# Leonhard111/M3L

Hardware: AMD Instinct MI355X
Metric: MAE fwd+bwd samples/sec (image+tactile) (higher is better)
Workload: dtype bf16; 1 GPU; BASELINE configs[1]: VTT vision+tactile MAE, 64x64 RGB + 2x32x32 tactile, ViT-Tiny 192/12/3/768 + decoder 192/4/3/768, mask 0.75; batch_per_gpu=256, global_batch=256, parallelism=dp1, grad_allreduce=none (one rank), rccl_ranks=0, step=zero_grad + mask + fwd + bwd + grad all-reduce + Adam

## Files before the change

include/m3l_amd.h:

```cpp
#ifndef M3L_AMD_H
#define M3L_AMD_H
#include <stddef.h>
#include <stdint.h>

#ifdef __cplusplus
extern "C" {
#endif

#define M3L_MAX_TACTILES 8

typedef struct m3l_geom {
    int image_h, image_w, image_patch, image_channels;
    int tactile_h, tactile_w, tactile_patch, tactile_channels;
    int num_tactiles;
    int use_vision;
    int use_tactile;
} m3l_geom;

typedef struct m3l_tf_cfg {
    int dim, depth, heads, mlp_dim;
    int project_out;
    int dtype;
    int dim_head;
} m3l_tf_cfg;
// ... 174 lines not shown
int m3l_prof_count(void);
int m3l_prof_get(int i, char* name, size_t n, double* ms_total, long* launches, double* flops_total, double* bytes_total);

int m3l_op_gemm_nt(int dtype, const void* A, int lda, const void* W, int ldw, int M, int N, int K, const float* bias,
                   const float* res, float* out_f32, void* out_t, void* out_pre, const void* gelu_u, int act, int ldc, void* stream);
size_t m3l_op_gemm_tn_ws_bytes(int M, int N, int K);
int m3l_op_gemm_tn(int dtype, const void* Y, int ldy, const void* X, int ldx, int M, int N, int K, void* ws, size_t ws_bytes,
                   float* out, int ldo, void* stream);
int m3l_op_gemm_tn_acc(int dtype, const void* Y, int ldy, const void* X, int ldx, int M, int N, int K, void* ws, size_t ws_bytes, float* out, int ldo,
                       int accumulate, void* stream);
size_t m3l_op_gemm_tn_grouped_ws_bytes(int dtype, int count, int M, const int* N, const int* K);
int m3l_op_gemm_tn_grouped(int dtype, int count, int M, const void* const* Y, const int* ldy, const void* const* X, const int* ldx, const int* N,
                           const int* K, float* const* out, void* ws, size_t ws_bytes, void* stream);
size_t m3l_op_colsum_ws_bytes(int N);
int m3l_op_colsum(int dtype, const void* Y, int M, int N, int ld, void* ws, float* out, void* stream);
int m3l_op_prep_weight(int dtype, const float* src, int rows, int cols, void* dst, void* dstT, void* stream);
int m3l_op_mask_scale(int mode, const float* src, const void* ref, float scale, long count, float* out, void* stream);
int m3l_op_concat2(float* a, int na, float* b, int nb, int rows, float* cat, int split, void* stream);
int m3l_op_patch_cols(int dtype, const float* x, int B, int C, int H, int W, int P, int Kpad, void* col, void* stream);
int m3l_op_vit_tokens(const float* emb, const float* cls, const float* regs, const float* pos, int B, int npatch, int R, int D, float* tok,
                      void* stream);
int m3l_op_attn_fwd(int dtype, const void* qkv, void* o, float* lse, int B, int n, int H, void* stream);
int m3l_op_attn_bwd(int dtype, const void* qkv, const void* o, const void* dO, const float* lse, float* dsum, void* dqkv, int B,
                    int n, int H, void* stream);
int m3l_op_attn_fwd_dh(int dtype, const void* qkv, void* o, float* lse, int B, int n, int H, void* stream, int dim_head);
int m3l_op_attn_bwd_dh(int dtype, const void* qkv, const void* o, const void* dO, const float* lse, float* dsum, void* dqkv, int B,
                       int n, int H, void* stream, int dim_head);
int m3l_op_dropout_mask(float p, uint64_t seed, int layer, int site, long rows, int N, uint8_t* out, void* stream);

int m3l_op_l2norm_fwd(int out_dtype, const float* x, int M, int D, float eps, void* y, float* y32, float* norm, void* stream);
// ... 34 lines not shown
```

m3l_amd/_lib.py:

```python
import ctypes as C
import os

_HERE = os.path.dirname(os.path.abspath(__file__))
LIB_PATH = os.environ.get("M3L_LIB_PATH") or os.path.join(_HERE, "lib", "libm3l_amd.so")

c_p = C.c_void_p
c_i = C.c_int
c_sz = C.c_size_t


class Geom(C.Structure):
    _fields_ = [(n, c_i) for n in ("image_h", "image_w", "image_patch", "image_channels", "tactile_h", "tactile_w",
                                   "tactile_patch", "tactile_channels", "num_tactiles", "use_vision", "use_tactile")]


class CnnCfg(C.Structure):
    _fields_ = [(n, c_i) for n in ("in_channels", "height", "width", "dim", "tactile", "dtype")]


class TfCfg(C.Structure):
    _fields_ = [(n, c_i) for n in ("dim", "depth", "heads", "mlp_dim", "project_out", "dtype", "dim_head")]


class MaeCfg(C.Structure):
# ... 92 lines not shown
    "m3l_adamw_step": (c_i, [c_p, c_p, c_p, c_p, C.c_long, C.c_float, C.c_float, C.c_float, C.c_float, C.c_float, c_i, C.c_float, C.c_float, c_p, c_i, c_p]),
    "m3l_adam_step": (c_i, [c_p, c_p, c_p, c_p, C.c_long, C.c_float, C.c_float, C.c_float, C.c_float, C.c_float, c_i, c_p]),
    "m3l_adam_step_scaled": (c_i, [c_p, c_p, c_p, c_p, C.c_long, C.c_float, C.c_float, C.c_float, C.c_float, C.c_float, c_i, C.c_float, c_p]),
    "m3l_dino_opt_step": (c_i, [c_p, c_p, c_p, c_p, c_p, C.c_long, c_p, c_p, c_i, C.POINTER(C.c_float), C.POINTER(C.c_float), c_i,
                                C.c_double, C.c_double, C.c_float, c_i, C.c_float, C.c_float, c_p, c_i, C.c_double, c_p]),
    "m3l_prof_begin": (None, [C.c_char_p, c_i]),
    "m3l_prof_end": (None, []),
    "m3l_prof_event_overhead_us": (C.c_double, [c_p, c_i]),
    "m3l_prof_count": (c_i, []),
    "m3l_prof_get": (c_i, [c_i, C.c_char_p, c_sz, C.POINTER(C.c_double), C.POINTER(C.c_long), C.POINTER(C.c_double),
                           C.POINTER(C.c_double)]),
    "m3l_op_gemm_nt": (c_i, [c_i, c_p, c_i, c_p, c_i, c_i, c_i, c_i, c_p, c_p, c_p, c_p, c_p, c_p, c_i, c_i, c_p]),
    "m3l_op_gemm_tn_ws_bytes": (c_sz, [c_i, c_i, c_i]),
    "m3l_op_gemm_tn": (c_i, [c_i, c_p, c_i, c_p, c_i, c_i, c_i, c_i, c_p, c_sz, c_p, c_i, c_p]),
    "m3l_op_gemm_tn_acc": (c_i, [c_i, c_p, c_i, c_p, c_i, c_i, c_i, c_i, c_p, c_sz, c_p, c_i, c_i, c_p]),
    "m3l_op_gemm_tn_grouped_ws_bytes": (c_sz, [c_i, c_i, c_i, c_p, c_p]),
    "m3l_op_gemm_tn_grouped": (c_i, [c_i, c_i, c_i, c_p, c_p, c_p, c_p, c_p, c_p, c_p, c_p, c_sz, c_p]),
    "m3l_op_colsum_ws_bytes": (c_sz, [c_i]),
    "m3l_op_colsum": (c_i, [c_i, c_p, c_i, c_i, c_i, c_p, c_p, c_p]),
    "m3l_op_prep_weight": (c_i, [c_i, c_p, c_i, c_i, c_p, c_p, c_p]),
    "m3l_op_mask_scale": (c_i, [c_i, c_p, c_p, C.c_float, C.c_long, c_p, c_p]),
    "m3l_op_concat2": (c_i, [c_p, c_i, c_p, c_i, c_i, c_p, c_i, c_p]),
    "m3l_op_patch_cols": (c_i, [c_i, c_p, c_i, c_i, c_i, c_i, c_i, c_i, c_p, c_p]),
    "m3l_op_vit_tokens": (c_i, [c_p, c_p, c_p, c_p, c_i, c_i, c_i, c_i, c_p, c_p]),
    "m3l_op_attn_fwd": (c_i, [c_i, c_p, c_p, c_p, c_i, c_i, c_i, c_p]),
    "m3l_op_attn_bwd": (c_i, [c_i, c_p, c_p, c_p, c_p, c_p, c_p, c_i, c_i, c_i, c_p]),
    "m3l_op_attn_fwd_dh": (c_i, [c_i, c_p, c_p, c_p, c_i, c_i, c_i, c_p, c_i]),
    "m3l_op_attn_bwd_dh": (c_i, [c_i, c_p, c_p, c_p, c_p, c_p, c_p, c_i, c_i, c_i, c_p, c_i]),
    "m3l_op_dropout_mask": (c_i, [C.c_float, C.c_uint64, c_i, c_i, C.c_long, c_i, c_p, c_p]),
    "m3l_op_l2norm_fwd": (c_i, [c_i, c_p, c_i, c_i, C.c_float, c_p, c_p, c_p, c_p]),
# ... 70 lines not shown
```

m3l_amd/csrc/elementwise.hip:

```cpp
#include "common.cuh"
#include "kernels.h"
#include <cstring>
#include <vector>

namespace {

constexpr int MAXV = 16;
constexpr int WPB = 4;

__device__ __forceinline__ void store_val(float* p, float v) { *p = v; }
__device__ __forceinline__ void store_val(bf16* p, float v) { *p = (bf16)v; }


template <typename TO> __device__ __forceinline__ void store4(TO* p, f32x4 v);
template <> __device__ __forceinline__ void store4<float>(float* p, f32x4 v) { *reinterpret_cast<f32x4*>(p) = v; }
template <> __device__ __forceinline__ void store4<bf16>(bf16* p, f32x4 v) {
    bf16x4 o;
    o[0] = (bf16)v[0]; o[1] = (bf16)v[1]; o[2] = (bf16)v[2]; o[3] = (bf16)v[3];
    *reinterpret_cast<bf16x4*>(p) = o;
}
__device__ __forceinline__ f32x4 load4(const float* p) { return *reinterpret_cast<const f32x4*>(p); }
__device__ __forceinline__ f32x4 load4(const bf16* p) {
    const bf16x4 v = *reinterpret_cast<const bf16x4*>(p);
    return f32x4{(float)v[0], (float)v[1], (float)v[2], (float)v[3]};
// ... 108 lines not shown
        if (256 * i >= D) break;
        *reinterpret_cast<f32x4*>(&red[wave][0][4 * lane]) = dg[i];
        *reinterpret_cast<f32x4*>(&red[wave][1][4 * lane]) = db[i];
        *reinterpret_cast<f32x4*>(&red[wave][2][4 * lane]) = dc[i];
        __syncthreads();
        const int e = 256 * i + threadIdx.x;
        if (e < D) {
#pragma unroll
            for (int k = 0; k < 3; ++k)
                out[k * D + e] = (red[0][k][threadIdx.x] + red[1][k][threadIdx.x]) + (red[2][k][threadIdx.x] + red[3][k][threadIdx.x]);
        }
        __syncthreads();
    }
}

__device__ __forceinline__ void reduce_cols_32x32(const float* __restrict__ p, int G, int stride, int j, bool valid,
                                                  float* __restrict__ out, int accumulate) {
    __shared__ float red[32][33];
    const int cl = threadIdx.x & 31, sl = threadIdx.x >> 5;
    float s = 0.f;
    if (valid) {
        float a[8] = {0.f, 0.f, 0.f, 0.f, 0.f, 0.f, 0.f, 0.f};
        int g = sl;
        for (; g + 224 < G; g += 256) {
#pragma unroll
            for (int u = 0; u < 8; ++u) a[u] += p[(long)(g + 32 * u) * stride + j];
        }
        for (; g < G; g += 32) a[0] += p[(long)g * stride + j];
        s = ((a[0] + a[1]) + (a[2] + a[3])) + ((a[4] + a[5]) + (a[6] + a[7]));
    }
    red[sl][cl] = s;
    __syncthreads();
    if (sl == 0 && valid) {
        float t = red[0][cl];
#pragma unroll
        for (int i = 1; i < 32; ++i) t += red[i][cl];
        out[j] = accumulate ? out[j] + t : t;
    }
}

__global__ __launch_bounds__(1024) void reduce_rows_kernel(const float* __restrict__ part, int G, int stride, int count,
                                                             float* __restrict__ out, int accumulate) {
    const int j = blockIdx.x * 32 + (threadIdx.x & 31);
    reduce_cols_32x32(part, G, stride, j, j < count, out, accumulate);
}

__global__ __launch_bounds__(1024) void reduce_vec_kernel(const float* __restrict__ v, int G, float* __restrict__ out, int accumulate) {
    __shared__ float red[16];
    float a0 = 0.f, a1 = 0.f, a2 = 0.f, a3 = 0.f;
    int i = threadIdx.x;
    for (; i + 3072 < G; i += 4096) { a0 += v[i]; a1 += v[i + 1024]; a2 += v[i + 2048]; a3 += v[i + 3072]; }
    for (; i < G; i += 1024) a0 += v[i];
    float s = wave_sum((a0 + a1) + (a2 + a3));
    if ((threadIdx.x & 63) == 0) red[threadIdx.x >> 6] = s;
    __syncthreads();
    if (threadIdx.x == 0) {
        float t = 0.f;
#pragma unroll
        for (int w = 0; w < 16; ++w) t += red[w];
        out[0] = accumulate ? out[0] + t : t;
    }
}

struct ReduceSegs { float* out[4]; };
__global__ __launch_bounds__(1024) void reduce_rows_seg_kernel(const float* __restrict__ part, int G, int stride, int width,
                                                                 ReduceSegs segs, int accumulate) {
    float* out = segs.out[blockIdx.y];
    if (!out) return;
    const int j = blockIdx.x * 32 + (threadIdx.x & 31);
    reduce_cols_32x32(part + (long)blockIdx.y * width, G, stride, j, j < width, out, accumulate);
}

__global__ __launch_bounds__(1024) void reduce_rows_batch_kernel(ReduceBatch b, int accumulate) {
    const ReduceBatchItem it = b.it[blockIdx.z];
    float* out = it.out[blockIdx.y];
    if (!out) return;
    const int j = blockIdx.x * 32 + (threadIdx.x & 31);
    reduce_cols_32x32(it.part + (long)blockIdx.y * b.D, it.G, 3 * b.D, j, j < b.D, out, accumulate);
}

template <typename T> struct Vec4;
template <> struct Vec4<bf16> { typedef bf16x4 type; };
template <> struct Vec4<float> { typedef f32x4 type; };
template <typename T>
__global__ __launch_bounds__(256) void colsum_kernel(const T* __restrict__ Y, int M, int N, int ld, int rows_per_block,
                                                       float* __restrict__ part, int vec_ok) {
    typedef typename Vec4<T>::type V4;
    const int r0 = blockIdx.x * rows_per_block, r1 = min(M, r0 + rows_per_block);
    for (int c = threadIdx.x * 4; c < N; c += 1024) {
        if (vec_ok && c + 4 <= N) {
            f32x4 s0 = f32x4{0.f, 0.f, 0.f, 0.f}, s1 = s0, s2 = s0, s3 = s0;
            auto ld4 = [&](int r) {
                const V4 v = *reinterpret_cast<const V4*>(Y + (long)r * ld + c);
// ... 1025 lines not shown
        else { if (D <= 256) LN_FWD(float, 1, bf16); else if (D <= 512) LN_FWD(float, 2, bf16); else LN_FWD(float, 4, bf16); }
    } else if (out_dtype == 1) {
        if (D <= 256) LN_FWD(bf16, 1, float); else if (D <= 512) LN_FWD(bf16, 2, float); else LN_FWD(bf16, 4, float);
    } else {
        if (D <= 256) LN_FWD(float, 1, float); else if (D <= 512) LN_FWD(float, 2, float); else LN_FWD(float, 4, float);
    }
#undef LN_FWD
    M3L_LAUNCH_CHECK();
    return 0;
}

int m3l_reduce_rows(const float* part, int G, int stride, int count, float* out, int accumulate, hipStream_t st) {
    if (count == 1 && stride == 1)
        reduce_vec_kernel<<<1, 1024, 0, st>>>(part, G, out, accumulate);
    else
        reduce_rows_kernel<<<cdiv(count, 32), 1024, 0, st>>>(part, G, stride, count, out, accumulate);
    M3L_LAUNCH_CHECK();
    return 0;
}

int m3l_ln_bwd_blocks(int M) {
    static const int forced = getenv("M3L_LN_ROWS_PER_WAVE") ? atoi(getenv("M3L_LN_ROWS_PER_WAVE")) : 0;
    const int rpw = forced > 0 ? forced : (M >= 12288 ? 4 : std::max(1, M / 4096));
    int G = cdiv(M, rpw * WPB);
    if (G > 2048) G = 2048;
    return G < 1 ? 1 : G;
}

int m3l_ln_bwd(int dy_dtype, const void* dy, const float* x, int M, int D, const float* gamma, float eps, const float* dres,
               float* dx_out, void* dx_t_out, int ct_dtype, float* part_ws, float* dgamma, float* dbeta, float* dbias,
               int accumulate, hipStream_t st) {
// ... 5 lines not shown
#define LN_BWD(TD, TC, C, TX) ln_bwd_kernel<TD, TC, C, TX><<<G, 256, 0, st>>>((const TD*)dy, (const TX*)x, M, D, gamma, eps, dres, dx_out, (TC*)dx_t_out, part_ws)
#define LN_BWD_C(TD, TC, TX) { if (D <= 256) LN_BWD(TD, TC, 1, TX); else if (D <= 512) LN_BWD(TD, TC, 2, TX); else LN_BWD(TD, TC, 4, TX); }
        if (m3l_call_rb()) {
            M3L_CHECK(!dx_out && dx_t_out && ct_dtype == 1, "ln_bwd: bf16 residual mode writes the compute-type gradient only");
            if (dy_dtype == 1) LN_BWD_C(bf16, bf16, bf16) else LN_BWD_C(float, bf16, bf16)
        }
        else if (dy_dtype == 1) LN_BWD_C(bf16, bf16, float)
        else if (ct_dtype == 1) LN_BWD_C(float, bf16, float)
        else LN_BWD_C(float, float, float)
#undef LN_BWD_C
#undef LN_BWD
    }
    M3L_LAUNCH_CHECK();
    if (!dgamma && !dbeta && !dbias) return 0;
    ReduceSegs segs = {{dgamma, dbeta, dbias, nullptr}};
    reduce_rows_seg_kernel<<<dim3(cdiv(D, 32), 3), 1024, 0, st>>>(part_ws, G, 3 * D, D, segs, accumulate);
    M3L_LAUNCH_CHECK();
    return 0;
}

int m3l_reduce_rows_batch(const ReduceBatch* b, int accumulate, hipStream_t st) {
    if (b->count <= 0) return 0;
    M3L_CHECK(b->count <= M3L_REDUCE_BATCH_MAX && b->D > 0, "reduce_rows_batch: count=%d D=%d", b->count, b->D);
    ProfScope prof("reduce_batch", b->count, b->D, 0, 0.0, st);
    reduce_rows_batch_kernel<<<dim3(cdiv(b->D, 32), 3, b->count), 1024, 0, st>>>(*b, accumulate);
    M3L_LAUNCH_CHECK();
    return 0;
}

int m3l_reduce_rows_seg3(const float* part, int G, int D, float* out0, float* out1, float* out2, int accumulate, hipStream_t st) {
    ReduceSegs segs = {{out0, out1, out2, nullptr}};
    reduce_rows_seg_kernel<<<dim3(cdiv(D, 32), 3), 1024, 0, st>>>(part, G, 3 * D, D, segs, accumulate);
    M3L_LAUNCH_CHECK();
    return 0;
}

int m3l_colsum(int dtype, const void* Y, int M, int N, int ld, float* part_ws, float* out, int accumulate, hipStream_t st) {
    M3L_CHECK(M > 0 && N > 0, "colsum: bad shape");
    int G = cdiv(M, N > 512 ? 16 : 64);
    if (G > m3l_part_blocks()) G = m3l_part_blocks();
    const int rpb = cdiv(M, G);
    G = cdiv(M, rpb);
    ProfScope prof("colsum", M, N, dtype, (double)M * N * (dtype ? 2 : 4), st);
    const int vec_ok = (ld % 4 == 0) && (N % 4 == 0) && (((unsigned long)Y) % 16 == 0) && (((unsigned long)part_ws) % 16 == 0);
    if (dtype == 1)
        colsum_kernel<bf16><<<G, 256, 0, st>>>((const bf16*)Y, M, N, ld, rpb, part_ws, vec_ok);
    else
// ... 137 lines not shown
int k_tokens_assemble(const float* img_tok, const float* tac_tok, int B, int D, int n_img, int n_tac, int k, const float* mod,
                        const float* pos_img, const float* pos_tac, float* tokens, hipStream_t st) {
    const long rows = (long)B * (n_img + k * n_tac);
    tokens_assemble_kernel<<<cdiv(rows, WPB), 256, 0, st>>>(img_tok, tac_tok, B, D, n_img, n_tac > 0 ? n_tac : 1, k, mod, pos_img, pos_tac, tokens);
    M3L_LAUNCH_CHECK();
    return 0;
}

int k_tokens_assemble_bwd(const float* dtok, int B, int D, int n_img, int n_tac, int k, float* d_img, float* d_tac, float* part_ws,
                            float* dmod, int accumulate, hipStream_t st) {
    const long rows = (long)B * (n_img + k * n_tac);
    const int PL = (1 + k) * D;
    const int G = part_grid(rows);
    tokens_assemble_bwd_kernel<<<G, 256, WPB * PL * sizeof(float), st>>>(dtok, B, D, n_img, n_tac > 0 ? n_tac : 1, k, d_img, d_tac, part_ws);
    M3L_LAUNCH_CHECK();
    reduce_rows_kernel<<<cdiv(PL, 32), 1024, 0, st>>>(part_ws, G, PL, PL, dmod, accumulate);
    M3L_LAUNCH_CHECK();
    return 0;
}

int m3l_adam_flat(float* p, const float* g, float* m, float* v, long n, float lr, float b1, float b2, float eps, float wd, int step,
                  float gscale, hipStream_t st) {
    M3L_CHECK(n > 0 && step >= 1, "adam: n=%ld step=%d", n, step);
    const float bc1 = 1.0f - powf(b1, (float)step);
    const float bc2_sqrt = sqrtf(1.0f - powf(b2, (float)step));
    adam_flat_kernel<0><<<cdiv(cdiv(n, 4), 256), 256, 0, st>>>(p, const_cast<float*>(g), m, v, n, lr, b1, b2, eps, wd, bc1, bc2_sqrt, nullptr, gscale, nullptr, 0);
    M3L_LAUNCH_CHECK();
    return 0;
}

int m3l_adamw_flat(float* p, float* g, float* m, float* v, long n, float lr, float b1, float b2, float eps, float wd, int step, float gscale,
// ... 181 lines not shown
    const int rows = B * cnt;
    if (rows == 0) return 0;
    const int pd = pg->C * pg->P * pg->P;
    const int G = part_grid(rows);
    const bool wide = pd > 64 * MAXV, tiny = pd <= 256;
    const int vec = pd % 4 == 0 && pdpad % 4 == 0 && aligned_to(dxn, 4 * (dtype == 1 ? 2 : 4));
#define PATCH_LN_BWD(T, NV) patch_ln_bwd_kernel<T, NV><<<G, 256, 0, st>>>(*pg, idx, idx_ld, j0, cnt, rows, eps, (const T*)dxn, pdpad, part_ws, vec)
    if (dtype == 1) {
        if (wide) PATCH_LN_BWD(bf16, PATCH_NV_MAX); else if (tiny) PATCH_LN_BWD(bf16, 4); else PATCH_LN_BWD(bf16, MAXV);
    } else {
        if (wide) PATCH_LN_BWD(float, PATCH_NV_MAX); else if (tiny) PATCH_LN_BWD(float, 4); else PATCH_LN_BWD(float, MAXV);
    }
#undef PATCH_LN_BWD
    M3L_LAUNCH_CHECK();
    ReduceSegs segs = {{dgamma, dbeta, nullptr, nullptr}};
    reduce_rows_seg_kernel<<<dim3(cdiv(pd, 32), 2), 1024, 0, st>>>(part_ws, G, 2 * pd, pd, segs, accumulate);
    M3L_LAUNCH_CHECK();
    return 0;
}

int m3l_embed_finalize(const float* E, int D, const PatchGroup* pg, const int64_t* idx, int idx_ld, int j0, int cnt, int B,
                       const float* gamma, const float* beta, float eps, const float* mod, int mod0, const float* pos,
                       float* tokens, int L, hipStream_t st) {
    const int rows = B * cnt;
    if (rows == 0) return 0;
    M3L_CHECK(D <= 64 * MAXV, "embed_finalize: D=%d too large", D);
    embed_finalize_kernel<<<ln_grid(rows), 256, 0, st>>>(E, rows, D, *pg, idx, idx_ld, j0, cnt, gamma, beta, eps, mod, mod0, pos, tokens, L);
    M3L_LAUNCH_CHECK();
    return 0;
}

// ... 1 lines not shown
                           int idx_ld, int j0, int cnt, int B, const float* gamma, float eps, void* dE, float* part_ws,
                           float* dgamma, float* dbeta, float* dmod, int mod0, int accumulate, hipStream_t st) {
    const int rows = B * cnt;
    if (rows == 0) return 0;
    const int nslot = pg->nsrc;
    const int PL = (2 + nslot) * D;
    const int G = part_grid(rows);
    if (dtype == 1)
        embed_finalize_bwd_kernel<bf16><<<G, 256, WPB * PL * sizeof(float), st>>>(dtok, L, E, rows, D, *pg, idx, idx_ld, j0, cnt, gamma, eps, (bf16*)dE, part_ws, nslot);
    else
        embed_finalize_bwd_kernel<float><<<G, 256, WPB * PL * sizeof(float), st>>>(dtok, L, E, rows, D, *pg, idx, idx_ld, j0, cnt, gamma, eps, (float*)dE, part_ws, nslot);
    M3L_LAUNCH_CHECK();
    if (nslot <= 2) {
        float* dm = dmod + (long)mod0 * D;
        ReduceSegs segs = {{dgamma, dbeta, dm, nslot > 1 ? dm + D : nullptr}};
        reduce_rows_seg_kernel<<<dim3(cdiv(D, 32), 2 + nslot), 1024, 0, st>>>(part_ws, G, PL, D, segs, accumulate);
    } else {
        reduce_rows_kernel<<<cdiv(D, 32), 1024, 0, st>>>(part_ws, G, PL, D, dgamma, accumulate);
        reduce_rows_kernel<<<cdiv(D, 32), 1024, 0, st>>>(part_ws + D, G, PL, D, dbeta, accumulate);
        reduce_rows_kernel<<<cdiv(nslot * D, 32), 1024, 0, st>>>(part_ws + 2 * D, G, PL, nslot * D, dmod + (long)mod0 * D, accumulate);
    }
    M3L_LAUNCH_CHECK();
    return 0;
}

int k_unshuffle_fwd(const float* src, const float* mask_token, const int64_t* unmasked, int nvis, const int64_t* masked,
                      int nmask, int B, int dd, int n_img, int n_tac, const float* dmod, const float* pos_img, const float* pos_tac,
                      float* dec_in, hipStream_t st) {
    const long rows = (long)B * (nvis + nmask);
    M3L_CHECK(dd % 4 == 0, "unshuffle_fwd: dd=%d must be a multiple of 4", dd);
    if (m3l_call_io())
        unshuffle_fwd_kernel<bf16><<<cdiv(rows, WPB), 256, 0, st>>>(src, mask_token, unmasked, nvis, masked, nmask, B, dd, n_img, n_tac > 0 ? n_tac : 1, dmod,
                                                                     pos_img, pos_tac, reinterpret_cast<bf16*>(dec_in));
    else
        unshuffle_fwd_kernel<float><<<cdiv(rows, WPB), 256, 0, st>>>(src, mask_token, unmasked, nvis, masked, nmask, B, dd, n_img, n_tac > 0 ? n_tac : 1, dmod,
// ... 13 lines not shown
    while (cdiv(cdiv(rows, rpw), WPB) > m3l_part_blocks()) rpw *= 2;
    const int G = cdiv(cdiv(rows, rpw), WPB);
    const int vpw = cdiv((long)B * nvis, (long)G * WPB);
    const int N = nvis + nmask, nt = n_tac > 0 ? n_tac : 1;
    const size_t lds = WPB * PL * sizeof(float);
#define UNSH_BWD(C, TI) unshuffle_bwd_kernel<C, TI><<<G, 256, lds, st>>>((const TI*)dY, unmasked, nvis, B, N, dd, n_img, nt, nmod, rpw, vpw, dsrc, part_ws)
    if (m3l_call_io()) {
        if (dd <= 256) UNSH_BWD(1, bf16); else if (dd <= 512) UNSH_BWD(2, bf16); else UNSH_BWD(4, bf16);
    } else {
        if (dd <= 256) UNSH_BWD(1, float); else if (dd <= 512) UNSH_BWD(2, float); else UNSH_BWD(4, float);
    }
#undef UNSH_BWD
    M3L_LAUNCH_CHECK();
    if (nmod <= 3) {
        ReduceSegs segs = {{dmask_token, ddmod, nmod > 1 ? ddmod + dd : nullptr, nmod > 2 ? ddmod + 2 * dd : nullptr}};
        reduce_rows_seg_kernel<<<dim3(cdiv(dd, 32), 1 + nmod), 1024, 0, st>>>(part_ws, G, PL, dd, segs, accumulate);
    } else {
        reduce_rows_kernel<<<cdiv(dd, 32), 1024, 0, st>>>(part_ws, G, PL, dd, dmask_token, accumulate);
        reduce_rows_kernel<<<cdiv(nmod * dd, 32), 1024, 0, st>>>(part_ws + dd, G, PL, nmod * dd, ddmod, accumulate);
    }
    M3L_LAUNCH_CHECK();
    return 0;
}

int m3l_gather_rows(int dtype, const void* src, int N, int D, const int64_t* idx, int idx_ld, int j0, int cnt, int B, void* dst,
                    hipStream_t st) {
    const int rows = B * cnt;
    if (rows == 0) return 0;
    if (dtype == 1)
        gather_rows_kernel<bf16><<<ln_grid(rows), 256, 0, st>>>((const bf16*)src, N, D, idx, idx_ld, j0, cnt, rows, (bf16*)dst);
    else
        gather_rows_kernel<float><<<ln_grid(rows), 256, 0, st>>>((const float*)src, N, D, idx, idx_ld, j0, cnt, rows, (float*)dst);
    M3L_LAUNCH_CHECK();
    return 0;
// ... 149 lines not shown
```

m3l_amd/csrc/kernels.h:

```cpp
#pragma once
#include <hip/hip_runtime.h>
#include <stddef.h>
#include <stdint.h>

#define M3L_MAX_SENSORS 8
#define M3L_MAX_PARTIAL_BLOCKS 2048


struct DropCtx {
    uint32_t thr;
    float scale;
    uint32_t k0, k1;
    uint32_t ctr2;
    int on;
};
DropCtx m3l_drop_ctx(float p, uint64_t seed, int layer, int site);

struct ProfScope {
    int idx;
    hipStream_t stream;
    ProfScope(const char* kind, long a, long b, long c, double work, hipStream_t st, double bytes = 0.0);
    ~ProfScope();
};

// ... 58 lines not shown
int m3l_gemm_nt_rowln(int dtype, int mode, const void* A, int lda, const void* W, int ldw, int M, int N, int K, const RowLnEpi* ep,
                      hipStream_t st);
constexpr int M3L_REDUCE_BATCH_MAX = 56;
struct ReduceBatchItem {
    const float* part;
    float* out[3];
    int G;
};
struct ReduceBatch {
    ReduceBatchItem it[M3L_REDUCE_BATCH_MAX];
    int count, D;
};
int m3l_reduce_rows_batch(const ReduceBatch* b, int accumulate, hipStream_t st);
int m3l_ln_bwd_blocks(int M);
int m3l_reduce_rows_seg3(const float* part, int G, int D, float* out0, float* out1, float* out2, int accumulate, hipStream_t st);

struct TnProblem {
    const void* Y;
    const void* X;
    int ldy, ldx, N, K;
    float* out;
    int ldo, nvalid, kvalid;
    int tile0;
    long part_off;
    int gelu_x;
};
struct TnGroup {
    TnProblem p[4];
    int count, tiles_total;
    const float* extra_part;
// ... 155 lines not shown
```

m3l_amd/csrc/mae_plan.hip:

```cpp
#include <stdarg.h>
#include <stdio.h>
#include <stdlib.h>
#include <string.h>

#include <algorithm>
#include <map>
#include <mutex>
#include <vector>

#include "../../include/m3l_amd.h"
#include "common.cuh"
#include "kernels.h"


namespace {

constexpr float LN_EPS = 1e-5f;

struct SideStream {
    hipStream_t s = nullptr;
    std::vector<hipEvent_t> ev;
    int next = 0;
};
std::mutex g_side_mu;
// ... 1584 lines not shown
}
int m3l_op_gemm_tn_grouped(int dtype, int count, int M, const void* const* Y, const int* ldy, const void* const* X, const int* ldx, const int* N,
                           const int* K, float* const* out, void* ws, size_t ws_bytes, void* stream) {
    M3L_CHECK(count >= 1 && count <= M3L_TN_MAX_PROBLEMS && Y && X && ldy && ldx && N && K && out && ws, "gemm_tn_grouped: bad arguments (count %d)", count);
    TnProblem pr[M3L_TN_MAX_PROBLEMS];
    memset(pr, 0, sizeof(pr));
    for (int i = 0; i < count; ++i) {
        pr[i].Y = Y[i]; pr[i].X = X[i]; pr[i].ldy = ldy[i]; pr[i].ldx = ldx[i]; pr[i].N = N[i]; pr[i].K = K[i];
        pr[i].out = out[i]; pr[i].ldo = K[i]; pr[i].nvalid = N[i]; pr[i].kvalid = K[i];
    }
    return m3l_gemm_tn_grouped(dtype, pr, count, M, (float*)ws, ws_bytes, 0, (hipStream_t)stream);
}
int m3l_op_colsum(int dtype, const void* Y, int M, int N, int ld, void* ws, float* out, void* stream) {
    return m3l_colsum(dtype, Y, M, N, ld, (float*)ws, out, 0, (hipStream_t)stream);
}
size_t m3l_op_colsum_ws_bytes(int N) { return (size_t)M3L_MAX_PARTIAL_BLOCKS * N * sizeof(float) + 256; }
int m3l_op_prep_weight(int dtype, const float* src, int rows, int cols, void* dst, void* dstT, void* stream) {
    WeightPack pk;
    memset(&pk, 0, sizeof(pk));
    pk.d[0] = WeightDesc{src, dst, dstT, rows, cols, cols, rows};
    pk.count = 1;
    return m3l_prep_weights(dtype, &pk, (hipStream_t)stream);
}
int m3l_op_mask_scale(int mode, const float* src, const void* ref, float scale, long count, float* out, void* stream) {
    return m3l_mask_scale(mode, src, ref, scale, count, out, (hipStream_t)stream);
}
int m3l_op_concat2(float* a, int na, float* b, int nb, int rows, float* cat, int split, void* stream) {
    return m3l_concat2(a, na, b, nb, rows, cat, split, (hipStream_t)stream);
}
int m3l_op_patch_cols(int dtype, const float* x, int B, int C, int H, int W, int P, int Kpad, void* col, void* stream) {
// ... 32 lines not shown
```

m3l_amd/csrc/wgrad.hip:

```cpp
#include <string.h>

#include <algorithm>

#include "common.cuh"
#include "kernels.h"

namespace {

typedef int int4v __attribute__((ext_vector_type(4)));

struct WgProb {
    const bf16* A;
    const bf16* B;
    float* out;
    int lda, ldb, a, b, so_a, so_b, avalid, bvalid;
    int tile0, tiles_b;
    int gelu_a, gelu_b;
};
struct WgExtra {
    const float* part;
    float* out;
    int G, width;
};
struct WgGroup {
// ... 14 lines not shown
        asm volatile("s_mov_b32 %0, m0\n\ts_mov_b32 m0, %3\n\ts_nop 0\n\tbuffer_load_dwordx4 %1, %2, 0 offen lds\n\ts_mov_b32 m0, %0"
                     : "=&s"(keep)
                     : "v"(voff), "s"(rsrc), "s"(lds_dst)
                     : "memory");
}
__device__ __forceinline__ int4v make_rsrc(const void* p, long bytes) {
    const unsigned long a = (unsigned long)p;
    int4v r;
    r[0] = __builtin_amdgcn_readfirstlane((int)(a & 0xffffffffu));
    r[1] = __builtin_amdgcn_readfirstlane((int)((a >> 32) & 0xffffu));
    r[2] = __builtin_amdgcn_readfirstlane((int)(bytes > 2147483647L ? 2147483647L : bytes));
    r[3] = __builtin_amdgcn_readfirstlane(0x00020000);
    return r;
}

__device__ __forceinline__ Frag<bf16> ldtr(const char* panel, int k0, int c0, int lane) {
    const int g = lane >> 4, i = lane & 15, q = i >> 2, p = i & 3;
    const int r0 = k0 + 4 * g + q;
    const int chunk = (c0 >> 3) + (p >> 1);
    const int x = ((chunk ^ (2 * ((r0 >> 1) & 3))) << 4) + (p & 1) * 8;
    typedef __attribute__((address_space(3))) bf16x4* lds_p;
    const bf16x4 lo = __builtin_amdgcn_ds_read_tr16_b64_v4bf16((lds_p)(panel + r0 * 128 + x));
    const bf16x4 hi = __builtin_amdgcn_ds_read_tr16_b64_v4bf16((lds_p)(panel + (r0 + 16) * 128 + x));
    Frag<bf16> f;
    f.v[0] = lo[0]; f.v[1] = lo[1]; f.v[2] = lo[2]; f.v[3] = lo[3];
    f.v[4] = hi[0]; f.v[5] = hi[1]; f.v[6] = hi[2]; f.v[7] = hi[3];
    return f;
}

#ifndef WG_ABL
#define WG_ABL 0
#endif
constexpr int WG_NST = 4;

__device__ __forceinline__ void wait_vm(int n) {
    switch (n) {
    case 0: asm volatile("s_waitcnt vmcnt(0)" ::: "memory"); break;
    case 1: asm volatile("s_waitcnt vmcnt(1)" ::: "memory"); break;
// ... 47 lines not shown
        voff[j] = (unsigned)(((long)(m_beg + row) * ld + col) * 2);
        pdst[j] = (unsigned)(panel * 4096 + rg * 1024);
    }
    const unsigned incA = (unsigned)(32 * pb.lda * 2), incB = (unsigned)(32 * pb.ldb * 2);
    const unsigned lds0 = (unsigned)(unsigned long)(__attribute__((address_space(3))) char*)smem;
    auto issue = [&](int t) {
        if (WG_ABL & 4) return;
        const unsigned base = lds0 + (t % WG_NST) * SLOT;
#pragma unroll
        for (int j = 0; j < JMAX; ++j) {
            if (!pv[j]) continue;
            if (pa[j]) dma16<NTL>(rsA, voff[j] + (unsigned)t * incA, __builtin_amdgcn_readfirstlane(base + pdst[j]));
            else dma16<NTL>(rsB, voff[j] + (unsigned)t * incB, __builtin_amdgcn_readfirstlane(base + pdst[j]));
        }
    };
    const bool work = a0 + 64 * wr < pb.a;

    f32x4 acc[4][NB];
#pragma unroll
    for (int x = 0; x < 4; ++x)
#pragma unroll
        for (int y = 0; y < NB; ++y) acc[x][y] = f32x4{0.f, 0.f, 0.f, 0.f};

    for (int t = 0; t < WG_NST - 1 && t < nst; ++t) issue(t);
    for (int t = 0; t < nst; ++t) {
        wait_vm(min(WG_NST - 2, nst - 1 - t) * mine);
        __builtin_amdgcn_s_barrier();
        asm volatile("" ::: "memory");
        if (t + WG_NST - 1 < nst) issue(t + WG_NST - 1);
        if (pb.gelu_a | pb.gelu_b) {
            char* base = smem + (t % WG_NST) * SLOT + (pb.gelu_a ? 0 : NA * 4096);
            const int bytes = pb.gelu_a ? NA * 4096 : TBT * 4096, form = pb.gelu_a | pb.gelu_b;
            for (int off = tid * 16; off < bytes; off += 64 * NW * 16) {
                bf16x8 v = *reinterpret_cast<bf16x8*>(base + off);
#pragma unroll
                for (int j = 0; j < 8; ++j) v[j] = (bf16)(form == 1 ? gelu_f((float)v[j]) : gelu_fast((float)v[j]));
                *reinterpret_cast<bf16x8*>(base + off) = v;
            }
            asm volatile("s_waitcnt lgkmcnt(0)" ::: "memory");
            __builtin_amdgcn_s_barrier();
        }
        if ((WG_ABL & 2) || !work) continue;
        const char* As = smem + (t % WG_NST) * SLOT + wr * 4096;
        const char* Bs = smem + (t % WG_NST) * SLOT + NA * 4096;
        Frag<bf16> fa[4], fb[NB];
#pragma unroll
        for (int x = 0; x < 4; ++x) fa[x] = ldtr(As, 0, x * 16, lane);
#pragma unroll
        for (int y = 0; y < NB; ++y) {
            const int col = wc * (TB / 2) + y * 16;
            fb[y] = ldtr(Bs + (col >> 6) * 4096, 0, col & 63, lane);
        }
        if (WG_ABL & 1) {
#pragma unroll
            for (int x = 0; x < 4; ++x) asm volatile("" ::"v"(fa[x].v));
#pragma unroll
            for (int y = 0; y < NB; ++y) asm volatile("" ::"v"(fb[y].v));
            continue;
        }
#pragma unroll
        for (int x = 0; x < 4; ++x)
#pragma unroll
            for (int y = 0; y < NB; ++y) acc[x][y] = mma16(fa[x], fb[y], acc[x][y]);
    }
    if (WG_ABL & 8) return;
    float* S = slabs + (long)w * (long)(TA * TB);
// ... 236 lines not shown
```

Baseline: 73330 samples/s.

## Shrink row-reduce blocks with batched loads; precompute LDS fragment offsets in wgrad

The column-sum reduction kernels drop from 1024-thread to 256-thread blocks. Each thread now covers several group rows, and all loads are issued before the adds so more memory requests are in flight. Separately, the wgrad GEMM computes each lane's LDS transpose-read offset once and derives per-fragment addresses with an XOR, which trims address arithmetic in the inner loop. New reduce_rows and reduce_rows_segs entry points are also exported; the tail handling in the reduction is more intricate and could mishandle edge cases.

```diff
diff --git a/include/m3l_amd.h b/include/m3l_amd.h
--- a/include/m3l_amd.h
+++ b/include/m3l_amd.h
@@ -212,6 +212,8 @@
                            const int* K, float* const* out, void* ws, size_t ws_bytes, void* stream);
 size_t m3l_op_colsum_ws_bytes(int N);
 int m3l_op_colsum(int dtype, const void* Y, int M, int N, int ld, void* ws, float* out, void* stream);
+int m3l_op_reduce_rows(const float* part, int G, int stride, int count, float* out, int accumulate, void* stream);
+int m3l_op_reduce_rows_segs(const float* part, int G, int stride, int width, int nseg, float* const* outs, int accumulate, void* stream);
 int m3l_op_prep_weight(int dtype, const float* src, int rows, int cols, void* dst, void* dstT, void* stream);
 int m3l_op_mask_scale(int mode, const float* src, const void* ref, float scale, long count, float* out, void* stream);
 int m3l_op_concat2(float* a, int na, float* b, int nb, int rows, float* cat, int split, void* stream);
diff --git a/m3l_amd/_lib.py b/m3l_amd/_lib.py
--- a/m3l_amd/_lib.py
+++ b/m3l_amd/_lib.py
@@ -130,6 +130,8 @@
     "m3l_op_gemm_tn_ws_bytes": (c_sz, [c_i, c_i, c_i]),
     "m3l_op_gemm_tn": (c_i, [c_i, c_p, c_i, c_p, c_i, c_i, c_i, c_i, c_p, c_sz, c_p, c_i, c_p]),
     "m3l_op_gemm_tn_acc": (c_i, [c_i, c_p, c_i, c_p, c_i, c_i, c_i, c_i, c_p, c_sz, c_p, c_i, c_i, c_p]),
+    "m3l_op_reduce_rows": (c_i, [c_p, c_i, c_i, c_i, c_p, c_i, c_p]),
+    "m3l_op_reduce_rows_segs": (c_i, [c_p, c_i, c_i, c_i, c_i, c_p, c_i, c_p]),
     "m3l_op_gemm_tn_grouped_ws_bytes": (c_sz, [c_i, c_i, c_i, c_p, c_p]),
     "m3l_op_gemm_tn_grouped": (c_i, [c_i, c_i, c_i, c_p, c_p, c_p, c_p, c_p, c_p, c_p, c_p, c_sz, c_p]),
     "m3l_op_colsum_ws_bytes": (c_sz, [c_i]),
diff --git a/m3l_amd/csrc/elementwise.hip b/m3l_amd/csrc/elementwise.hip
--- a/m3l_amd/csrc/elementwise.hip
+++ b/m3l_amd/csrc/elementwise.hip
@@ -146,24 +146,56 @@
     }
 }
 
+template <int TS>
 __device__ __forceinline__ void reduce_cols_32x32(const float* __restrict__ p, int G, int stride, int j, bool valid,
                                                   float* __restrict__ out, int accumulate) {
+    constexpr int NU = 32 / TS;
     __shared__ float red[32][33];
-    const int cl = threadIdx.x & 31, sl = threadIdx.x >> 5;
-    float s = 0.f;
+    const int cl = threadIdx.x & 31, ts = threadIdx.x >> 5;
     if (valid) {
-        float a[8] = {0.f, 0.f, 0.f, 0.f, 0.f, 0.f, 0.f, 0.f};
-        int g = sl;
-        for (; g + 224 < G; g += 256) {
-#pragma unroll
-            for (int u = 0; u < 8; ++u) a[u] += p[(long)(g + 32 * u) * stride + j];
-        }
-        for (; g < G; g += 32) a[0] += p[(long)g * stride + j];
-        s = ((a[0] + a[1]) + (a[2] + a[3])) + ((a[4] + a[5]) + (a[6] + a[7]));
-    }
-    red[sl][cl] = s;
+        float a[NU][8];
+#pragma unroll
+        for (int u = 0; u < NU; ++u)
+#pragma unroll
+            for (int k = 0; k < 8; ++k) a[u][k] = 0.f;
+        int g = ts;
+        for (; g + TS * (NU - 1) + 224 < G; g += 256) {
+            float t[NU][8];
+#pragma unroll
+            for (int u = 0; u < NU; ++u)
+#pragma unroll
+                for (int k = 0; k < 8; ++k) t[u][k] = p[(long)(g + TS * u + 32 * k) * stride + j];
+            asm volatile("" ::: "memory");
+#pragma unroll
+            for (int u = 0; u < NU; ++u)
+#pragma unroll
+                for (int k = 0; k < 8; ++k) a[u][k] += t[u][k];
+        }
+#pragma unroll
+        for (int u = 0; u < NU; ++u) {
+            const int gu = g + TS * u;
+            if (gu < G) {
+                float t[8];
+#pragma unroll
+                for (int k = 0; k < 8; ++k) t[k] = p[(long)min(gu + 32 * k, G - 1) * stride + j];
+                asm volatile("" ::: "memory");
+                if (gu + 224 < G) {
+#pragma unroll
+                    for (int k = 0; k < 8; ++k) a[u][k] += t[k];
+                } else {
+#pragma unroll
+                    for (int k = 0; k < 7; ++k)
+                        if (gu + 32 * k < G) a[u][0] += t[k];
+                }
+            }
+            red[ts + TS * u][cl] = ((a[u][0] + a[u][1]) + (a[u][2] + a[u][3])) + ((a[u][4] + a[u][5]) + (a[u][6] + a[u][7]));
+        }
+    } else {
+#pragma unroll
+        for (int u = 0; u < NU; ++u) red[ts + TS * u][cl] = 0.f;
+    }
     __syncthreads();
-    if (sl == 0 && valid) {
+    if (ts == 0 && valid) {
         float t = red[0][cl];
 #pragma unroll
         for (int i = 1; i < 32; ++i) t += red[i][cl];
@@ -171,10 +203,11 @@
     }
 }
 
-__global__ __launch_bounds__(1024) void reduce_rows_kernel(const float* __restrict__ part, int G, int stride, int count,
-                                                             float* __restrict__ out, int accumulate) {
+constexpr int RR_TS = 8, RR_THREADS = 32 * RR_TS;
+__global__ __launch_bounds__(RR_THREADS) void reduce_rows_kernel(const float* __restrict__ part, int G, int stride, int count,
+                                                                   float* __restrict__ out, int accumulate) {
     const int j = blockIdx.x * 32 + (threadIdx.x & 31);
-    reduce_cols_32x32(part, G, stride, j, j < count, out, accumulate);
+    reduce_cols_32x32<RR_TS>(part, G, stride, j, j < count, out, accumulate);
 }
 
 __global__ __launch_bounds__(1024) void reduce_vec_kernel(const float* __restrict__ v, int G, float* __restrict__ out, int accumulate) {
@@ -195,12 +228,12 @@
 }
 
 struct ReduceSegs { float* out[4]; };
-__global__ __launch_bounds__(1024) void reduce_rows_seg_kernel(const float* __restrict__ part, int G, int stride, int width,
-                                                                 ReduceSegs segs, int accumulate) {
+__global__ __launch_bounds__(RR_THREADS) void reduce_rows_seg_kernel(const float* __restrict__ part, int G, int stride, int width,
+                                                                       ReduceSegs segs, int accumulate) {
     float* out = segs.out[blockIdx.y];
     if (!out) return;
     const int j = blockIdx.x * 32 + (threadIdx.x & 31);
-    reduce_cols_32x32(part + (long)blockIdx.y * width, G, stride, j, j < width, out, accumulate);
+    reduce_cols_32x32<RR_TS>(part + (long)blockIdx.y * width, G, stride, j, j < width, out, accumulate);
 }
 
 __global__ __launch_bounds__(1024) void reduce_rows_batch_kernel(ReduceBatch b, int accumulate) {
@@ -208,7 +241,7 @@
     float* out = it.out[blockIdx.y];
     if (!out) return;
     const int j = blockIdx.x * 32 + (threadIdx.x & 31);
-    reduce_cols_32x32(it.part + (long)blockIdx.y * b.D, it.G, 3 * b.D, j, j < b.D, out, accumulate);
+    reduce_cols_32x32<32>(it.part + (long)blockIdx.y * b.D, it.G, 3 * b.D, j, j < b.D, out, accumulate);
 }
 
 template <typename T> struct Vec4;
@@ -1264,7 +1297,7 @@
     if (count == 1 && stride == 1)
         reduce_vec_kernel<<<1, 1024, 0, st>>>(part, G, out, accumulate);
     else
-        reduce_rows_kernel<<<cdiv(count, 32), 1024, 0, st>>>(part, G, stride, count, out, accumulate);
+        reduce_rows_kernel<<<cdiv(count, 32), RR_THREADS, 0, st>>>(part, G, stride, count, out, accumulate);
     M3L_LAUNCH_CHECK();
     return 0;
 }
@@ -1300,7 +1333,7 @@
     M3L_LAUNCH_CHECK();
     if (!dgamma && !dbeta && !dbias) return 0;
     ReduceSegs segs = {{dgamma, dbeta, dbias, nullptr}};
-    reduce_rows_seg_kernel<<<dim3(cdiv(D, 32), 3), 1024, 0, st>>>(part_ws, G, 3 * D, D, segs, accumulate);
+    reduce_rows_seg_kernel<<<dim3(cdiv(D, 32), 3), RR_THREADS, 0, st>>>(part_ws, G, 3 * D, D, segs, accumulate);
     M3L_LAUNCH_CHECK();
     return 0;
 }
@@ -1316,7 +1349,17 @@
 
 int m3l_reduce_rows_seg3(const float* part, int G, int D, float* out0, float* out1, float* out2, int accumulate, hipStream_t st) {
     ReduceSegs segs = {{out0, out1, out2, nullptr}};
-    reduce_rows_seg_kernel<<<dim3(cdiv(D, 32), 3), 1024, 0, st>>>(part, G, 3 * D, D, segs, accumulate);
+    reduce_rows_seg_kernel<<<dim3(cdiv(D, 32), 3), RR_THREADS, 0, st>>>(part, G, 3 * D, D, segs, accumulate);
+    M3L_LAUNCH_CHECK();
+    return 0;
+}
+
+int m3l_reduce_rows_segs(const float* part, int G, int stride, int width, int nseg, float* const* outs, int accumulate, hipStream_t st) {
+    M3L_CHECK(nseg >= 1 && nseg <= 4 && G > 0 && width > 0 && stride >= nseg * width, "reduce_rows_segs: nseg=%d G=%d width=%d stride=%d", nseg, G,
+              width, stride);
+    ReduceSegs segs = {{nullptr, nullptr, nullptr, nullptr}};
+    for (int i = 0; i < nseg; ++i) segs.out[i] = outs[i];
+    reduce_rows_seg_kernel<<<dim3(cdiv(width, 32), nseg), RR_THREADS, 0, st>>>(part, G, stride, width, segs, accumulate);
     M3L_LAUNCH_CHECK();
     return 0;
 }
@@ -1484,7 +1527,7 @@
     const int G = part_grid(rows);
     tokens_assemble_bwd_kernel<<<G, 256, WPB * PL * sizeof(float), st>>>(dtok, B, D, n_img, n_tac > 0 ? n_tac : 1, k, d_img, d_tac, part_ws);
     M3L_LAUNCH_CHECK();
-    reduce_rows_kernel<<<cdiv(PL, 32), 1024, 0, st>>>(part_ws, G, PL, PL, dmod, accumulate);
+    reduce_rows_kernel<<<cdiv(PL, 32), RR_THREADS, 0, st>>>(part_ws, G, PL, PL, dmod, accumulate);
     M3L_LAUNCH_CHECK();
     return 0;
 }
@@ -1696,7 +1739,7 @@
 #undef PATCH_LN_BWD
     M3L_LAUNCH_CHECK();
     ReduceSegs segs = {{dgamma, dbeta, nullptr, nullptr}};
-    reduce_rows_seg_kernel<<<dim3(cdiv(pd, 32), 2), 1024, 0, st>>>(part_ws, G, 2 * pd, pd, segs, accumulate);
+    reduce_rows_seg_kernel<<<dim3(cdiv(pd, 32), 2), RR_THREADS, 0, st>>>(part_ws, G, 2 * pd, pd, segs, accumulate);
     M3L_LAUNCH_CHECK();
     return 0;
 }
@@ -1728,11 +1771,11 @@
     if (nslot <= 2) {
         float* dm = dmod + (long)mod0 * D;
         ReduceSegs segs = {{dgamma, dbeta, dm, nslot > 1 ? dm + D : nullptr}};
-        reduce_rows_seg_kernel<<<dim3(cdiv(D, 32), 2 + nslot), 1024, 0, st>>>(part_ws, G, PL, D, segs, accumulate);
+        reduce_rows_seg_kernel<<<dim3(cdiv(D, 32), 2 + nslot), RR_THREADS, 0, st>>>(part_ws, G, PL, D, segs, accumulate);
     } else {
-        reduce_rows_kernel<<<cdiv(D, 32), 1024, 0, st>>>(part_ws, G, PL, D, dgamma, accumulate);
-        reduce_rows_kernel<<<cdiv(D, 32), 1024, 0, st>>>(part_ws + D, G, PL, D, dbeta, accumulate);
-        reduce_rows_kernel<<<cdiv(nslot * D, 32), 1024, 0, st>>>(part_ws + 2 * D, G, PL, nslot * D, dmod + (long)mod0 * D, accumulate);
+        reduce_rows_kernel<<<cdiv(D, 32), RR_THREADS, 0, st>>>(part_ws, G, PL, D, dgamma, accumulate);
+        reduce_rows_kernel<<<cdiv(D, 32), RR_THREADS, 0, st>>>(part_ws + D, G, PL, D, dbeta, accumulate);
+        reduce_rows_kernel<<<cdiv(nslot * D, 32), RR_THREADS, 0, st>>>(part_ws + 2 * D, G, PL, nslot * D, dmod + (long)mod0 * D, accumulate);
     }
     M3L_LAUNCH_CHECK();
     return 0;
@@ -1776,10 +1819,10 @@
     M3L_LAUNCH_CHECK();
     if (nmod <= 3) {
         ReduceSegs segs = {{dmask_token, ddmod, nmod > 1 ? ddmod + dd : nullptr, nmod > 2 ? ddmod + 2 * dd : nullptr}};
-        reduce_rows_seg_kernel<<<dim3(cdiv(dd, 32), 1 + nmod), 1024, 0, st>>>(part_ws, G, PL, dd, segs, accumulate);
+        reduce_rows_seg_kernel<<<dim3(cdiv(dd, 32), 1 + nmod), RR_THREADS, 0, st>>>(part_ws, G, PL, dd, segs, accumulate);
     } else {
-        reduce_rows_kernel<<<cdiv(dd, 32), 1024, 0, st>>>(part_ws, G, PL, dd, dmask_token, accumulate);
-        reduce_rows_kernel<<<cdiv(nmod * dd, 32), 1024, 0, st>>>(part_ws + dd, G, PL, nmod * dd, ddmod, accumulate);
+        reduce_rows_kernel<<<cdiv(dd, 32), RR_THREADS, 0, st>>>(part_ws, G, PL, dd, dmask_token, accumulate);
+        reduce_rows_kernel<<<cdiv(nmod * dd, 32), RR_THREADS, 0, st>>>(part_ws + dd, G, PL, nmod * dd, ddmod, accumulate);
     }
     M3L_LAUNCH_CHECK();
     return 0;
diff --git a/m3l_amd/csrc/kernels.h b/m3l_amd/csrc/kernels.h
--- a/m3l_amd/csrc/kernels.h
+++ b/m3l_amd/csrc/kernels.h
@@ -96,6 +96,7 @@
 int m3l_reduce_rows_batch(const ReduceBatch* b, int accumulate, hipStream_t st);
 int m3l_ln_bwd_blocks(int M);
 int m3l_reduce_rows_seg3(const float* part, int G, int D, float* out0, float* out1, float* out2, int accumulate, hipStream_t st);
+int m3l_reduce_rows_segs(const float* part, int G, int stride, int width, int nseg, float* const* outs, int accumulate, hipStream_t st);
 
 struct TnProblem {
     const void* Y;
diff --git a/m3l_amd/csrc/mae_plan.hip b/m3l_amd/csrc/mae_plan.hip
--- a/m3l_amd/csrc/mae_plan.hip
+++ b/m3l_amd/csrc/mae_plan.hip
@@ -1622,6 +1622,13 @@
 int m3l_op_colsum(int dtype, const void* Y, int M, int N, int ld, void* ws, float* out, void* stream) {
     return m3l_colsum(dtype, Y, M, N, ld, (float*)ws, out, 0, (hipStream_t)stream);
 }
+int m3l_op_reduce_rows(const float* part, int G, int stride, int count, float* out, int accumulate, void* stream) {
+    M3L_CHECK(G > 0 && count > 0 && stride >= count, "reduce_rows: G=%d count=%d stride=%d", G, count, stride);
+    return m3l_reduce_rows(part, G, stride, count, out, accumulate, (hipStream_t)stream);
+}
+int m3l_op_reduce_rows_segs(const float* part, int G, int stride, int width, int nseg, float* const* outs, int accumulate, void* stream) {
+    return m3l_reduce_rows_segs(part, G, stride, width, nseg, outs, accumulate, (hipStream_t)stream);
+}
 size_t m3l_op_colsum_ws_bytes(int N) { return (size_t)M3L_MAX_PARTIAL_BLOCKS * N * sizeof(float) + 256; }
 int m3l_op_prep_weight(int dtype, const float* src, int rows, int cols, void* dst, void* dstT, void* stream) {
     WeightPack pk;
diff --git a/m3l_amd/csrc/wgrad.hip b/m3l_amd/csrc/wgrad.hip
--- a/m3l_amd/csrc/wgrad.hip
+++ b/m3l_amd/csrc/wgrad.hip
@@ -52,14 +52,16 @@
     return r;
 }
 
-__device__ __forceinline__ Frag<bf16> ldtr(const char* panel, int k0, int c0, int lane) {
+__device__ __forceinline__ unsigned frag_lane(int lane) {
     const int g = lane >> 4, i = lane & 15, q = i >> 2, p = i & 3;
-    const int r0 = k0 + 4 * g + q;
-    const int chunk = (c0 >> 3) + (p >> 1);
-    const int x = ((chunk ^ (2 * ((r0 >> 1) & 3))) << 4) + (p & 1) * 8;
+    const int r0 = 4 * g + q;
+    return (unsigned)(r0 * 128 + (((r0 >> 1) & 3) << 5) + (p >> 1) * 16 + (p & 1) * 8);
+}
+__device__ __forceinline__ Frag<bf16> ldtr(unsigned lds0, unsigned off, int cx) {
     typedef __attribute__((address_space(3))) bf16x4* lds_p;
-    const bf16x4 lo = __builtin_amdgcn_ds_read_tr16_b64_v4bf16((lds_p)(panel + r0 * 128 + x));
-    const bf16x4 hi = __builtin_amdgcn_ds_read_tr16_b64_v4bf16((lds_p)(panel + (r0 + 16) * 128 + x));
+    const unsigned a = lds0 + (off ^ ((unsigned)cx << 5));
+    const bf16x4 lo = __builtin_amdgcn_ds_read_tr16_b64_v4bf16((lds_p)(unsigned long)a);
+    const bf16x4 hi = __builtin_amdgcn_ds_read_tr16_b64_v4bf16((lds_p)(unsigned long)(a + 16 * 128));
     Frag<bf16> f;
     f.v[0] = lo[0]; f.v[1] = lo[1]; f.v[2] = lo[2]; f.v[3] = lo[3];
     f.v[4] = hi[0]; f.v[5] = hi[1]; f.v[6] = hi[2]; f.v[7] = hi[3];
@@ -137,6 +139,7 @@
             else dma16<NTL>(rsB, voff[j] + (unsigned)t * incB, __builtin_amdgcn_readfirstlane(base + pdst[j]));
         }
     };
+    const unsigned lfrag = frag_lane(lane);
     const bool work = a0 + 64 * wr < pb.a;
 
     f32x4 acc[4][NB];
@@ -164,15 +167,15 @@
             __builtin_amdgcn_s_barrier();
         }
         if ((WG_ABL & 2) || !work) continue;
-        const char* As = smem + (t % WG_NST) * SLOT + wr * 4096;
-        const char* Bs = smem + (t % WG_NST) * SLOT + NA * 4096;
+        const unsigned so = (unsigned)((t % WG_NST) * SLOT);
+        const unsigned offA = (so + wr * 4096) + lfrag;
         Frag<bf16> fa[4], fb[NB];
 #pragma unroll
-        for (int x = 0; x < 4; ++x) fa[x] = ldtr(As, 0, x * 16, lane);
+        for (int x = 0; x < 4; ++x) fa[x] = ldtr(lds0, offA, x);
 #pragma unroll
         for (int y = 0; y < NB; ++y) {
             const int col = wc * (TB / 2) + y * 16;
-            fb[y] = ldtr(Bs + (col >> 6) * 4096, 0, col & 63, lane);
+            fb[y] = ldtr(lds0, (so + (NA + (col >> 6)) * 4096) + lfrag, (col >> 4) & 3);
         }
         if (WG_ABL & 1) {
 #pragma unroll
```

Measured after the change: 70210 samples/s. 0.957x the previous value.
